# gaoxiang12/ORB-YGZ-SLAM

Hardware: AMD Instinct MI355X
Metric: frames/s ORB extract+match, 752x480 8-lvl 1000-feat; 1->8 GPU scaling (higher is better)
Workload: dtype u8

## Files before the change

### orb_ygz_slam_amd/csrc/extract_kernels.hip

```cpp
#include <cstdlib>

#include <cstring>
#include <mutex>
#include "kernels.h"
#include "wave_ops.h"
#include "describe_lds.h"
#include "fast9_quad.h"
#include "fast_lane_quads.h"
#include "orb_pattern_table.h"

namespace ygzf {

typedef short v2s __attribute__((ext_vector_type(2)));
typedef unsigned short v2u __attribute__((ext_vector_type(2)));

__device__ __forceinline__ int lane_id() { return threadIdx.x & 63; }
__device__ __forceinline__ int wave_id() { return __builtin_amdgcn_readfirstlane(threadIdx.x >> 6); }

#ifdef YGZF_PHASE_CLOCK
constexpr int kPhaseSlots = 8192;
__device__ unsigned g_phase_rec[2][kPhaseSlots][10];
struct PhaseClk {
    unsigned long long t;
    unsigned a[8], extra;
// ... 98 lines not shown
    __syncthreads();
    const unsigned long long total = tmp64[16];
    unsigned long long off = tmp64[wave_id()] + incl - s;
    for (int i = lo; i < hi; i++) {
        const unsigned long long v = (unsigned long long) (unsigned) a[i] | ((unsigned long long) (unsigned) b[i] << 21) | ((unsigned long long) (unsigned) c[i] << 42);
        a[i] = (int) (off & 0x1FFFFFu); b[i] = (int) ((off >> 21) & 0x1FFFFFu); c[i] = (int) (off >> 42);
        off += v;
    }
    __syncthreads();
    *totA = (int) (total & 0x1FFFFFu); *totB = (int) ((total >> 21) & 0x1FFFFFu); *totC = (int) (total >> 42);
}

constexpr int kRadixBits = 7;
constexpr int radix_hist_ints(int waves) { return (1 << kRadixBits) * waves; }
template <int kWaves>
__device__ void block_radix_sort(unsigned *k0, unsigned *v0, unsigned *k1, unsigned *v1, int n, int bits,
                                 volatile int *histT, int *tmp, unsigned **rk, unsigned **rv) {
    static_assert(kWaves >= 1 && kWaves <= 16, "block_excl_scan's scratch holds up to 16 waves");
    const int lane = lane_id(), wave = wave_id();
    constexpr int nw = kWaves;
    const int seg = (((n + nw - 1) / nw) + 63) & ~63;
    const int start = wave * seg;
    const int end = min(n, start + seg);
    const unsigned long long lt = (1ull << lane) - 1ull;
    constexpr int NB = 1 << kRadixBits;
    for (int shift = 0; shift < bits; shift += kRadixBits) {
        for (int t = threadIdx.x; t < NB * nw; t += blockDim.x) histT[t] = 0;
        __syncthreads();
        for (int i = start + lane; i < end; i += 64) {
            const int d = (k0[i] >> shift) & (NB - 1);
            atomicAdd((int *) &histT[d * nw + wave], 1);
        }
        __syncthreads();
        block_scan_array((int *) histT, NB * nw, tmp);
        for (int base = start; base < end; base += 64) {
            const int i = base + lane;
            const bool valid = i < end;
            const unsigned key = valid ? k0[i] : 0u;
            const unsigned val = valid ? v0[i] : 0u;
            const int d = (key >> shift) & (NB - 1);
            unsigned long long m = __ballot(valid);
// ... 945 lines not shown
    int tid, l, f, parts, part;
    LevelGeom g;
    OctShared S;
    int nCells, passEv;
    int *PS;
    unsigned *candB;
    unsigned *xTab;
    const unsigned short *cc;
    const unsigned *sl;
    unsigned *key0, *val0, *key1, *val1, *xy;
    int dm, nBins, binShift;
    int *lvlCnt, *gd, *gh;
    int *histT, *tmp, *flagA, *overflow, *cut, *head;
    unsigned long long *tmp64;
    bool hist, inLds;
    int M;
    unsigned *skeys, *svals;
    int n, cur, nE;
};

enum OctOutcome { kOctDone, kOctLeft, kOctAgainAlone, kOctAgainSorted };
__device__ __forceinline__ void oct_stamp(const OctLevel &w, long long *dbg, int k) {
    if (dbg && w.tid == 0 && w.f == 0 && w.part == 0) dbg[w.l * 8 + k] = wall_clock64();
}
__device__ __forceinline__ void oct_pass_stamp(OctLevel &w, long long *dbg, int nn) {
#ifdef YGZF_PHASE_CLOCK
    if (dbg && w.tid == 0 && w.f == 0 && w.part == 0 && w.passEv < 8) { dbg[16 * 8 + 16 + w.l * 16 + 2 * w.passEv] = nn; dbg[16 * 8 + 16 + w.l * 16 + 2 * w.passEv + 1] = wall_clock64(); w.passEv++; }
#endif
}
__device__ __forceinline__ void oct_helper_leaves(const OctLevel &w) {
// ... 23 lines not shown
    if (kGlobalNodes) S.cand = (unsigned *) dyn + Y.ints;
    else if (!kHist) S.cand = (unsigned *) dyn + oct_lds_sort_cand((int) (p - dyn), a.ldsCand);
    w.xTab = (unsigned *) (kGlobalNodes ? S.nlo[0] : dyn + Y.xTab);
}

template <int kBlock> __device__ __forceinline__ int oct_cell_prefix(const OctArgs &a, const OctLevel &w) {
    const OctShared &S = w.S;
    for (int i = w.tid; i < w.nCells; i += kBlock) S.cellPref[i] = w.cc[i];
    __syncthreads();
    const int M = block_scan_array(S.cellPref, w.nCells, w.tmp);
    if (w.tid == 0) { S.cellPref[w.nCells] = M; if (w.part == 0) a.lvlCandCnt[w.f * a.nlevels + w.l] = M; }
    __syncthreads();
    return M;
}

template <int kBlock> __device__ __forceinline__ void oct_key_tables(const OctLevel &w, int lenX, int lenY) {
    const LevelGeom &g = w.g;
    unsigned *xTab = w.xTab, *yTab = xTab + lenX, *orgTab = yTab + lenY;
    auto spread = [](unsigned v) {
        v = (v | (v << 8)) & 0x00FF00FFu;
        v = (v | (v << 4)) & 0x0F0F0F0Fu;
        v = (v | (v << 2)) & 0x33333333u;
        return (v | (v << 1)) & 0x55555555u;
    };
    auto halvings = [&](int v, int lo, int hi) {
        unsigned k = 0;
        for (int d = 0; d < g.depth; d++) {
            const int m = lo + ((hi - lo + 1) >> 1);
            const unsigned b = v >= m;
            if (b) lo = m; else hi = m;
            k = (k << 1) | b;
        }
        return k;
    };
    for (int t = w.tid; t < lenX + lenY + w.nCells; t += kBlock) {
        if (t < lenX) {
            const int root = min((int) ((float) t / g.hX), g.nIni - 1);
            xTab[t] = ((unsigned) root << (2 * g.depth)) | spread(halvings(t, (int) (g.hX * (float) root), (int) (g.hX * (float) (root + 1))));
        } else if (t < lenX + lenY) {
            yTab[t - lenX] = spread(halvings(t - lenX, 0, g.regH)) << 1;
        } else {
            const int c = t - lenX - lenY;
            const int ci = c / g.nCols, cj = c - ci * g.nCols;
            orgTab[c] = (unsigned) (cj * g.wCell) | ((unsigned) (ci * g.hCell) << 16);
        }
    }
    __syncthreads();
}

template <int kBlock> __device__ __forceinline__ void oct_path_keys(const OctLevel &w, bool useTab, int lenX, int lenY, int shares) {
    const LevelGeom &g = w.g; const OctShared &S = w.S;
    const int tid = w.tid, M = w.M, nCells = w.nCells;
    const unsigned *xTab = w.xTab, *yTab = xTab + lenX, *orgTab = yTab + lenY;
    int steps = 0;
    while ((1 << steps) < nCells) steps++;
    constexpr int kKU = 4;
    for (int i0 = tid + w.part * kKU * kBlock; i0 < M; i0 += shares * kKU * kBlock) {
        int ia[kKU], a[kKU], b[kKU];
#pragma unroll
        for (int u = 0; u < kKU; u++) { ia[u] = min(i0 + u * kBlock, M - 1); a[u] = 0; b[u] = nCells; }
        for (int st = 0; st < steps; st++) {
// ... 79 lines not shown
        int v = w.PS[b];
        for (int q = 0; q < w.parts - 1; q++) v += w.gh[(long long) q * a.histBins + b];
        w.PS[b] = v;
    }
    return kOctDone;
}

template <int kBlock> __device__ __forceinline__ void oct_order(OctLevel &w) {
    w.skeys = w.key0; w.svals = w.val0;
    if (w.hist) {
        block_scan_array(w.PS, w.nBins, w.tmp);
        if (w.tid == 0) w.PS[w.nBins] = w.M;
        __syncthreads();
    } else {
        unsigned *sk, *sv;
        block_radix_sort<kBlock / 64>(w.key0, w.val0, w.key1, w.val1, w.M, w.g.keyBits, w.histT, w.tmp, &sk, &sv);
        w.skeys = sk; w.svals = sv;
        if (w.inLds && w.candB && w.skeys == w.key1) {
            for (int i = w.tid; i < w.M; i += kBlock) { w.key0[i] = w.key1[i]; w.val0[i] = w.val1[i]; }
            __syncthreads();
            w.skeys = w.key0; w.svals = w.val0;
        }
    }
}

__device__ __forceinline__ int oct_first_bin(const int *PS, int nBins, int sh, int lo) {
    int a = 0, b = nBins >> sh;
    while (b - a > 1) {
        const int m = (a + b) >> 1;
        if (PS[m << sh] <= lo) a = m; else b = m;
    }
    return a << sh;
}
__device__ __forceinline__ void oct_bounds(const OctLevel &w, int lo, int cnt, int dep, int *a1, int *a2, int *a3) {
    if (w.hist) {
        if (dep + 1 > w.dm) {
            *w.overflow = 1;
            *a1 = *a2 = *a3 = lo + cnt;
            return;
        }
        const int sh = 2 * (w.dm - dep);
        const int f0 = oct_first_bin(w.PS, w.nBins, sh, lo), s1 = 1 << (sh - 2);
        *a1 = w.PS[f0 + s1]; *a2 = w.PS[f0 + 2 * s1]; *a3 = w.PS[f0 + 3 * s1];
    } else
        digit_bounds3(w.skeys, lo, cnt, 2 * (w.g.depth - (dep + 1)), a1, a2, a3);
}
__device__ __forceinline__ void oct_child_counts(int lo, int a1, int a2, int a3, int hi, int *k, int *e) {
    const int c0 = a1 - lo, c1 = a2 - a1, c2 = a3 - a2, c3 = hi - a3;
    *k = (c0 > 0) + (c1 > 0) + (c2 > 0) + (c3 > 0);
    *e = (c0 > 1) + (c1 > 1) + (c2 > 1) + (c3 > 1);
}
template <typename T> __device__ __forceinline__ void oct_place_children(const OctNodes &out, int lo, int cnt, int dep, int a1, int a2, int a3, int p, T *ePos, T *eCnt, int es) {
    const int bb[5] = {lo, a1, a2, a3, lo + cnt};
    int epos[4];
    for (int c = 3; c >= 0; c--) {
        const int cc2 = bb[c + 1] - bb[c];
        epos[c] = p;
        if (cc2 > 0) { out.lo[p] = bb[c]; out.cnt[p] = cc2; out.dep[p] = dep + 1; p++; }
    }
    for (int c = 0; c < 4; c++) {
        const int cc2 = bb[c + 1] - bb[c];
        if (cc2 > 1) { ePos[es] = (T) epos[c]; eCnt[es] = (T) cc2; es++; }
    }
}
__device__ __forceinline__ void oct_emit(const OctShared &S, const OctNodes &out, int lo, int cnt, int dep, int a1, int a2, int a3, int exK, int exE, int exS, int sumK) {
    if (cnt == 1) {
        const int p = sumK + exS;
        out.lo[p] = lo; out.cnt[p] = 1; out.dep[p] = dep;
    } else {
        int k, e;
        oct_child_counts(lo, a1, a2, a3, lo + cnt, &k, &e);
        oct_place_children(out, lo, cnt, dep, a1, a2, a3, sumK - (exK + k), S.Epos, S.Ecnt, exE);
    }
}
// ... 124 lines not shown
}

template <int kBlock> __device__ __forceinline__ void oct_expand_round(OctLevel &w) {
    const OctShared &S = w.S; const OctNodes in = oct_nodes(S, w.cur);
    const int tid = w.tid, n = w.n, nE = w.nE, N = w.g.nFeat;
    int seqBits = 1, cntBits = 1;
    while ((1 << seqBits) < max(nE, 2)) seqBits++;
    while ((1 << cntBits) <= w.M) cntBits++;
    for (int j = tid; j < nE; j += kBlock) { S.sk[0][j] = ((unsigned) S.Ecnt[j] << seqBits) | (unsigned) j; S.sv[0][j] = (unsigned) j; }
    for (int j = tid; j < n; j += kBlock) S.flag[j] = 0;
    if (tid == 0) *w.cut = nE - 1;
    __syncthreads();
    unsigned *ek, *ev;
    if (nE <= kBlock) { oct_rank_sort<kBlock>(w, nE); ek = S.sk[1]; ev = S.sv[1]; }
    else
        block_radix_sort<kBlock / 64>(S.sk[0], S.sv[0], S.sk[1], S.sv[1], nE, seqBits + cntBits, w.histT, w.tmp, &ek, &ev);
    for (int j = tid; j < nE; j += kBlock) {
        const int pos = S.Epos[(int) ev[nE - 1 - j]];
        const int cnt = in.cnt[pos], lo = in.lo[pos];
        int a1, a2, a3, k, e;
        oct_bounds(w, lo, cnt, in.dep[pos], &a1, &a2, &a3);
        S.b1[j] = a1; S.b2[j] = a2; S.b3[j] = a3;
        oct_child_counts(lo, a1, a2, a3, lo + cnt, &k, &e);
        S.kArr[j] = k - 1; S.eArr[j] = e;
    }
    __syncthreads();
    block_scan_array(S.kArr, nE, w.tmp);
    auto children = [&](int j) {
        const int pos = S.Epos[(int) ev[nE - 1 - j]];
        const int cnt = in.cnt[pos], lo = in.lo[pos];
        int k, e;
// ... 49 lines not shown
        const int prevSize = w.n;
        oct_full_pass<kBlock>(w);
        oct_pass_stamp(w, dbg, w.n);
        if (w.n >= N || w.n == prevSize) finish = true;
        else if (w.n + 3 * w.nE > N) toExpand = true;
    }
    while (!finish) {
        const int prevSize = w.n;
        if (w.nE == 0) break;
        oct_expand_round<kBlock>(w);
        oct_pass_stamp(w, dbg, -w.n);
        if (w.n >= N || w.n == prevSize) finish = true;
    }
}

template <bool kHist, int kBlock> __device__ __forceinline__ OctOutcome oct_attempt(const OctArgs &a, OctLevel &w, bool useHist, bool alone) {
    const LevelGeom &g = w.g; const int tid = w.tid;
    w.hist = kHist && useHist;
    if (kHist && tid == 0) *w.overflow = 0;
    w.M = oct_cell_prefix<kBlock>(a, w);
    if (w.M == 0) { oct_empty_level<kBlock>(a, w); return kOctLeft; }
    oct_stamp(w, a.dbg, 1);
    w.inLds = w.M <= a.ldsCand;
    if (w.inLds) {
        w.key0 = w.S.cand; w.val0 = w.S.cand + a.ldsCand;
        if (w.candB) { w.key1 = w.candB; w.val1 = w.candB + a.ldsCand; }
        else { w.key1 = w.S.cand + 2 * a.ldsCand; w.val1 = w.S.cand + 3 * a.ldsCand; }
    }
    const int lenX = max(g.regW, g.nCols * g.wCell) + 9, lenY = max(g.regH, g.nRows * g.hCell) + 9;
    const bool useTab = lenX + lenY + w.nCells <= oct_lds_tab_room(kHist, w.nCells, a.cap, a.regionInts) && g.depth <= 15;
    if (useTab) oct_key_tables<kBlock>(w, lenX, lenY);
    if (w.hist) {
        for (int b = tid; b <= w.nBins; b += kBlock) w.PS[b] = 0;
        __syncthreads();
    }
    const bool shared = w.hist && w.parts > 1 && !alone;
    oct_path_keys<kBlock>(w, useTab, lenX, lenY, shared ? w.parts : 1);
    if (shared) {
        const OctOutcome o = oct_hand_over<kBlock>(a, w);
        if (o != kOctDone) return o;
    }
    __syncthreads();
    oct_stamp(w, a.dbg, 2);
    oct_order<kBlock>(w);
    oct_stamp(w, a.dbg, 3);
    oct_subdivide<kBlock>(w, a.dbg);
    if (w.hist && *w.overflow) {
        __syncthreads();
        if (a.dbg && tid == 0) atomicAdd((unsigned long long *) &a.dbg[16 * 8 + w.l], 1ull);
        return kOctAgainSorted;
    }
    return kOctDone;
}

template <int kBlock> __device__ __forceinline__ void oct_best_hist(const OctLevel &w) {
    const OctShared &S = w.S; const OctNodes in = oct_nodes(S, w.cur);
    const int tid = w.tid, n = w.n, M = w.M, lane = lane_id(), wave = wave_id();
    int *PS = w.PS;
    for (int i = tid; i < n; i += kBlock) {
        const int sh = 2 * (w.dm - in.dep[i]);
        S.b1[i] = oct_first_bin(PS, w.nBins, sh, in.lo[i]);
// ... 32 lines not shown
        const bool ok = i < n;
        const int lo = ok ? in.lo[i] : 0, cnt = ok ? in.cnt[i] : 0;
        unsigned best = 0;
        for (int k = sl16; k < cnt; k += 16) best = max(best, w.svals[lo + k]);
        best = max(best, (unsigned) __builtin_amdgcn_update_dpp(0, (int) best, 0xB1, 0xF, 0xF, true));
        best = max(best, (unsigned) __builtin_amdgcn_update_dpp(0, (int) best, 0x4E, 0xF, 0xF, true));
        best = max(best, (unsigned) __builtin_amdgcn_update_dpp(0, (int) best, 0x141, 0xF, 0xF, true));
        best = max(best, (unsigned) __builtin_amdgcn_update_dpp(0, (int) best, 0x140, 0xF, 0xF, true));
        if (ok && sl16 == 0) S.kArr[i] = (int) best;
    }
}

template <int kBlock> __device__ __forceinline__ void oct_emit_keypoints(const OctArgs &a, const OctLevel &w) {
    const OctShared &S = w.S; const LevelGeom &g = w.g;
    const int tid = w.tid, n = w.n;
    unsigned *oxy = a.lvlKpXY + (long long) w.f * a.kpStride + g.kpBase;
    unsigned char *osc = a.lvlKpScore + (long long) w.f * a.kpStride + g.kpBase;
    for (int i = tid; i < n; i += kBlock) {
        const unsigned best = (unsigned) S.kArr[i];
        const unsigned idx = 0xFFFFFFu - (best & 0xFFFFFFu);
        const unsigned p = w.xy[idx];
        const unsigned kx = (p & 0xFFFFu) + kBorder, ky = (p >> 16) + kBorder;
        oxy[i] = kx | (ky << 16);
        osc[i] = (unsigned char) (best >> 24);
        S.b1[i] = (int) (kx | (ky << 16));
        S.b2[i] = (int) (best >> 24);
        S.sk[0][i] = ((ky >> 6) << 6) | (kx >> 6);
        S.sv[0][i] = (unsigned) i;
    }
    __syncthreads();
    unsigned *ok = S.sk[0], *ov = S.sv[0];
    if (gridDim.y > 4) block_radix_sort<kBlock / 64>(S.sk[0], S.sv[0], S.sk[1], S.sv[1], n, 12, w.histT, w.tmp, &ok, &ov);
    uint2 *pr = a.procRec + (long long) w.f * a.kpStride + g.kpBase;
    for (int i = tid; i < g.kpCap; i += kBlock) {
        if (i < n) {
            const unsigned li = ov[i];
            pr[i] = make_uint2((unsigned) S.b1[li], (unsigned) S.b2[li] | (li << 8) | ((unsigned) w.l << 24));
        } else pr[i] = make_uint2(0u, kNoKeypoint);
    }
    if (tid == 0) *w.lvlCnt = n;
}

template <bool kGlobalNodes, bool kHist, int kBlock>
__global__ __launch_bounds__(kBlock) __attribute__((amdgpu_waves_per_eu(kHist ? 4 : 8, 8))) void k_octree(OctArgs a) {
    static_assert(!(kGlobalNodes && kHist), "the histogram plan keeps the node arrays in LDS");
    extern __shared__ __attribute__((aligned(16))) int dyn[];
    __shared__ int histT[radix_hist_ints(kBlock / 64)];
// ... 13 lines not shown
    w.gd = kHist && w.parts > 1 ? a.gDone + (w.f * a.nlevels + w.l) : nullptr;
    w.gh = kHist && w.parts > 1 ? a.gHist + ((long long) w.f * a.nlevels + w.l) * (w.parts - 1) * a.histBins : nullptr;
    if (w.nCells <= 0 || g.nCols <= 0) { oct_empty_level<kBlock>(a, w); return; }
    oct_carve<kGlobalNodes, kHist>(a, w, dyn);
    w.cc = a.cellCnt + (long long) w.f * a.totalCells + g.cellBase;
    w.sl = a.slots + (long long) w.f * a.totalSlots + g.slotBase;
    const long long cand = (long long) w.f * a.candStride + g.candBase;
    w.key0 = a.candKey0 + cand; w.val0 = a.candVal0 + cand; w.key1 = a.candKey1 + cand; w.val1 = a.candVal1 + cand; w.xy = a.candXY + cand;
    w.dm = 0;
    if (kHist) {
        w.dm = g.depth;
        while (w.dm > 0 && ((long long) g.nIni << (2 * w.dm)) > (long long) a.histBins) w.dm--;
    }
    w.nBins = g.nIni << (2 * w.dm);
    w.binShift = 2 * (g.depth - w.dm);
    bool useHist = kHist && w.dm >= 1, alone = false;
    if (w.part != 0 && !useHist) { oct_helper_leaves(w); return; }
    for (;;) {
        const OctOutcome o = oct_attempt<kHist, kBlock>(a, w, useHist, alone);
        if (o == kOctLeft) return;
        if (o == kOctDone) break;
        if (o == kOctAgainAlone) alone = true;
        else useHist = false;
    }
    oct_stamp(w, a.dbg, 4);
    if (w.hist) oct_best_hist<kBlock>(w);
    else oct_best_sorted<kBlock>(w);
    __syncthreads();
    oct_emit_keypoints<kBlock>(a, w);
    oct_stamp(w, a.dbg, 5);
    if (a.dbg && w.tid == 0 && w.f == 0) { a.dbg[w.l * 8 + 6] = w.M; a.dbg[w.l * 8 + 7] = w.n; }
}

__device__ __forceinline__ float fast_atan2_deg(float y, float x) {
    const float k = (float) (180.0 / 3.14159265358979323846);
    const float p1 = 0.9997878412794807f * k, p3 = -0.3258083974640975f * k, p5 = 0.1555786518463281f * k,
                p7 = -0.04432655554792128f * k;
    const float ax = fabsf(x), ay = fabsf(y);
// ... 556 lines not shown
    else
        hipLaunchKernelGGL((k_fast_tab_persist<false>), grid, block, lds, st, fs, dCells, iniTh, minTh, cellCnt, slots, totalCells, totalSlots, recsPerFrame, magic,
                           totalItems, perXcd, winRows, smapRows, quadCap, stats, counters);
}

hipError_t octree_prepare(size_t ldsBytes, bool globalNodes, bool hist) {
    constexpr int kOctMaxDyn = 160 * 1024 - 10 * 1024;
    if (hist) return hipFuncSetAttribute((const void *) k_octree<false, true, kOctBlock>, hipFuncAttributeMaxDynamicSharedMemorySize, kOctMaxDyn);
    if (globalNodes) return hipFuncSetAttribute((const void *) k_octree<true, false, kOctBlock>, hipFuncAttributeMaxDynamicSharedMemorySize, kOctMaxDyn);
    hipError_t e = hipFuncSetAttribute((const void *) k_octree<false, false, 1024>, hipFuncAttributeMaxDynamicSharedMemorySize, kOctMaxDyn);
    if (e == hipSuccess) e = hipFuncSetAttribute((const void *) k_octree<false, false, 512>, hipFuncAttributeMaxDynamicSharedMemorySize, kOctMaxDyn);
    if (e == hipSuccess) e = hipFuncSetAttribute((const void *) k_octree<false, false, 256>, hipFuncAttributeMaxDynamicSharedMemorySize, kOctMaxDyn);
    return e;
}

void launch_octree(hipStream_t st, const OctArgs &a, int nLaunchLevels, int nFrames, size_t ldsBytes, int block, int helpers) {
    const dim3 grid(nLaunchLevels, nFrames, helpers);
    switch (a.histBins > 0 ? 1 : a.nodeArena ? 2 : block) {
        case 1: hipLaunchKernelGGL((k_octree<false, true, kOctBlock>), grid, dim3(kOctBlock), ldsBytes, st, a); break;
        case 2: hipLaunchKernelGGL((k_octree<true, false, kOctBlock>), grid, dim3(kOctBlock), ldsBytes, st, a); break;
        case 256: hipLaunchKernelGGL((k_octree<false, false, 256>), grid, dim3(256), ldsBytes, st, a); break;
        case 512: hipLaunchKernelGGL((k_octree<false, false, 512>), grid, dim3(512), ldsBytes, st, a); break;
        default: hipLaunchKernelGGL((k_octree<false, false, 1024>), grid, dim3(1024), ldsBytes, st, a); break;
    }
}

void launch_describe(hipStream_t st, const FrameSet &fs, const LevelGeom *dGeom, int nlevels, const int *lvlKpCnt, int *lvlBase,
                     const uint2 *procRec, int kpStride, ygzf_kp *outKp, uint8_t *outDesc, int *outCnt, int outStride, int nFrames, int cvMode) {
    const bool own = nFrames <= 4;
    if (!own) hipLaunchKernelGGL(k_level_bases, dim3((nFrames + 255) / 256), dim3(256), 0, st, lvlKpCnt, nlevels, nFrames, lvlBase, outCnt);
// ... 80 lines not shown
```

### orb_ygz_slam_amd/csrc/kernels.h

```cpp
#ifndef YGZF_KERNELS_H
#define YGZF_KERNELS_H
#include "ygzf_internal.h"
#include "ygzf_remap_plan.h"
#include "lds_layout.h"

namespace ygzf {

hipError_t upload_constants(const int *umax16);

struct PyrTabs {
    const int *xofs;
    const short *xalpha;
    const int *yofs;
    const short *ybeta;
    const PyrColRec *cols;
    const PyrRowRec *rows;
    const PyrTileRec *tiles;
};
void launch_pyr_resize(hipStream_t st, const FrameSet &fs, const LevelGeom *dGeom, const LevelGeom &g, int level, int nFrames, const PyrTabs &T);
constexpr int kPyrFolds = 4;
__host__ __device__ constexpr int pyr_fold_chunks(int foldLog2) { return foldLog2 == 0 ? 21 : foldLog2 == 1 ? 11 : foldLog2 == 2 ? 6 : 3; }
__host__ __device__ constexpr int pyr_fold_pitch(int foldLog2) { return 16 * pyr_fold_chunks(foldLog2); }
__host__ __device__ constexpr int pyr_fold_rows(int foldLog2) { return foldLog2 == 0 ? 44 : foldLog2 == 1 ? 84 : foldLog2 == 2 ? 166 : 330; }
constexpr int kPyrTileRows = 32;
// ... 32 lines not shown
void launch_pack_results(hipStream_t st, const int *cnt, const ygzf_kp *kp, const uint8_t *desc, int nFrames, int kpStride, void *dst, size_t offKp, size_t offDesc);
void launch_pack_levels(hipStream_t st, const FrameSet &fs, const LevelGeom *dGeom, int firstLevel, int nlevels, const unsigned *offsets, uint8_t *dst);
void launch_fast_cells(hipStream_t st, const FrameSet &fs, const LevelGeom *dGeom, int nlevels, int iniTh, int minTh,
                       unsigned short *cellCnt, unsigned *slots, int totalCells, long long totalSlots, int totalGroups, int smapRows,
                       int nFrames, int winPitch, int winRows, int quadCap, const int *groupBaseHost, bool iniFirst, unsigned *stats);
constexpr int kFastTabMaxCell = 41;
void launch_fast_tab(hipStream_t st, const FrameSet &fs, const FastCellRec *dCells, int iniTh, int minTh, unsigned short *cellCnt, unsigned *slots,
                     int totalCells, long long totalSlots, int totalGroups, int smapRows, int nFrames, int winRows, int quadCap, bool iniFirst,
                     unsigned *stats);
hipError_t phase_clocks_read(int kernel, unsigned long long *out16, bool reset);
constexpr size_t kFastPersistCounterBytes = 64 * 256;
void launch_fast_tab_persist(hipStream_t st, const FrameSet &fs, const FastCellRec *dCells, int iniTh, int minTh, unsigned short *cellCnt, unsigned *slots,
                             int totalCells, long long totalSlots, int totalGroups, int smapRows, int nFrames, int winRows, int quadCap, bool iniFirst,
                             unsigned *stats, unsigned *counters, int nWorkgroups);
constexpr int kFastStatWords = 8 * 64;
int octree_lds_cand(int maxCellsPerLevel, int cap, size_t budget);
hipError_t octree_prepare(size_t ldsBytes, bool globalNodes, bool hist);
struct OctArgs {
    const LevelGeom *geom;
    int nlevels, levelBase;
    const unsigned short *cellCnt;
    const unsigned *slots;
    int totalCells;
    long long totalSlots;
    unsigned *candKey0, *candVal0, *candKey1, *candVal1, *candXY;
    long long candStride;
    unsigned *lvlKpXY;
    unsigned char *lvlKpScore;
    int *lvlKpCnt, *lvlCandCnt;
    uint2 *procRec;
    int kpStride;
    int cap, ldsCand;
    int *nodeArena;
    int regionInts, histBins;
    int *gHist, *gDone;
    int doneTarget, spinBudget;
    long long *dbg;
};
void launch_octree(hipStream_t st, const OctArgs &a, int nLaunchLevels, int nFrames, size_t ldsBytes, int block, int helpers);
constexpr int kOctDbgAlone = 16 * 8 + 16 + 16 * 16;
constexpr int kOctDbgAloneFrames = kOctDbgAlone + 16;
constexpr int kOctDbgWords = kOctDbgAloneFrames + 1;
void launch_describe(hipStream_t st, const FrameSet &fs, const LevelGeom *dGeom, int nlevels, const int *lvlKpCnt, int *lvlBase,
                     const uint2 *procRec, int kpStride, ygzf_kp *outKp, uint8_t *outDesc, int *outCnt, int outStride, int nFrames, int cvMode);
void launch_hamming_pairs(hipStream_t st, const void *a, const void *b, int n, int *out);

struct MatchQueryScratch;
struct MatchArgs {
// ... 374 lines not shown
```

### orb_ygz_slam_amd/csrc/ygzf_api.hip

```cpp
#include <cmath>
#include <cstdarg>
#include <cstdio>
#include <cstdlib>
#include <cstring>
#include <limits>
#include <mutex>

#include "ygzf_ctx.h"

using namespace ygzf;

thread_local std::string g_create_err;

int apply_geometry(ygzf_ctx *c, int w, int h, int nFrames) {
    if (w < 1 || h < 1) return fail(c, YGZF_ERR_INVALID, "image size %dx%d", w, h);
    if (w > c->maxW || h > c->maxH) return fail(c, YGZF_ERR_INVALID, "image %dx%d exceeds the context maximum %dx%d", w, h, c->maxW, c->maxH);
    if (nFrames < 1 || nFrames > c->maxBatch) return fail(c, YGZF_ERR_INVALID, "batch of %d frames (context maximum %d)", nFrames, c->maxBatch);
    const int L = c->tab.cfg.nlevels;
    if (c->geo.w != w || c->geo.h != h) {
        Geometry G;
        OctPlan oct;
        std::string msg;
        int rc = build_geometry(c->tab, c->pins, w, h, G, &msg);
        if (!rc) rc = plan_octree(G, L, c->pins, oct, &msg);
// ... 37 lines not shown
                for (size_t q = 0; q < rel.size(); q++) {
                    std::memset(&rel[q], 0, sizeof rel[q]);
                    for (int l = G.pyrBase; l < L; l++) rel[q].lv[l - G.pyrBase] = G.pyrPlan[q].lv[l];
                }
                HIPCHECK(c, hipMemcpy(c->dPyrPlan.p, lv, sizeof lv, hipMemcpyHostToDevice));
                HIPCHECK(c, hipMemcpy((char *) c->dPyrPlan.p + sizeof G.pyrLevels, rel.data(), rel.size() * sizeof(PyrStripPlan), hipMemcpyHostToDevice));
            }
            if (pyr_strips_prepare(G.pyrStripLds) != hipSuccess) {
                (void) hipGetLastError();
                G.pyrPlan.clear();
            }
        }
        rc = ensure(c, c->dFastCells, std::max<size_t>(G.fastCells.size() * sizeof(FastCellRec), 32));
        if (rc) return rc;
        if (!G.fastCells.empty()) HIPCHECK(c, hipMemcpy(c->dFastCells.p, G.fastCells.data(), G.fastCells.size() * sizeof(FastCellRec), hipMemcpyHostToDevice));
        if (oct.haveSmall || oct.kind == OctPlan::Hist) HIPCHECK(c, octree_prepare(0, false, true));
        if (oct.kind != OctPlan::Hist) HIPCHECK(c, octree_prepare(oct.launches[0].lds, oct.launches[0].arena, false));
        c->oct = oct;
        c->geo = G;
    }
    const Geometry &G = c->geo;
    const size_t B = (size_t) nFrames;
    int rc = 0;
    const size_t oldPyr = c->dPyr.bytes;
    rc = ensure(c, c->dPyr, std::max<size_t>(B * G.pyrBytes, 16) + 256);
    if (oldPyr != c->dPyr.bytes) forget_image(c);
    if (rc) return rc;
    if ((rc = ensure(c, c->dCellCnt, std::max<size_t>(B * G.totalCells * sizeof(unsigned short), 16)))) return rc;
    if ((rc = ensure(c, c->dSlots, std::max<size_t>(B * G.totalSlots * sizeof(unsigned), 16)))) return rc;
    const size_t cb = std::max<size_t>(B * G.candStride * sizeof(unsigned), 16);
// ... 127 lines not shown
    }
    if (collect) HIPCHECK(c, hipMemcpyAsync(c->hFastStats, c->dFastStats.p, kFastStatWords * sizeof(unsigned), hipMemcpyDeviceToHost, c->stream));
    return YGZF_OK;
}

static OctArgs oct_args(const ygzf_ctx *c, const OctLaunch &grp, long long *odbg) {
    const Geometry &G = c->geo;
    OctArgs a{};
    a.geom = (const LevelGeom *) c->dGeom.p; a.nlevels = c->tab.cfg.nlevels; a.levelBase = grp.l0; a.cap = grp.cap; a.dbg = odbg;
    a.cellCnt = (const unsigned short *) c->dCellCnt.p; a.slots = (const unsigned *) c->dSlots.p; a.totalCells = G.totalCells; a.totalSlots = G.totalSlots;
    a.candKey0 = (unsigned *) c->dK0.p; a.candVal0 = (unsigned *) c->dV0.p; a.candKey1 = (unsigned *) c->dK1.p; a.candVal1 = (unsigned *) c->dV1.p;
    a.candXY = (unsigned *) c->dXY.p; a.candStride = G.candStride; a.procRec = (uint2 *) c->dProcOrder.p; a.kpStride = G.kpStride;
    a.lvlKpXY = (unsigned *) c->dLvlXY.p; a.lvlKpScore = (unsigned char *) c->dLvlScore.p; a.lvlKpCnt = (int *) c->dLvlCnt.p; a.lvlCandCnt = (int *) c->dLvlCand.p;
    a.ldsCand = grp.ldsCand; a.regionInts = grp.regionInts; a.histBins = grp.histBins;
    a.nodeArena = grp.arena ? (int *) c->dOctNodes.p : nullptr;
    return a;
}

static int arm_oct_helpers(ygzf_ctx *c, int nFrames, int L, const OctLaunch &small, OctArgs *a, int *helpersOut) {
    const Geometry &G = c->geo;
    int helpers = c->pins.octHelpers;
    if (helpers < 0) helpers = G.totalCells >= 2000 ? std::min(8, std::max(1, c->cuCount) / std::max(1, nFrames * L)) : 1;
    helpers = std::max(1, std::min(helpers, std::min(8, std::max(1, c->cuCount / std::max(1, nFrames * L)))));
    if (helpers > 1) {
        const size_t words = (size_t) nFrames * L * (helpers - 1) * small.histBins, bytes = (words + 64) * sizeof(int) + (size_t) nFrames * L * sizeof(int);
        int rcH = ensure(c, c->dOctHist, bytes);
        if (rcH) return rcH;
        const ygzf_ctx::OctHistLayout lay{nFrames, helpers, small.histBins, c->dOctHist.bytes};
        if (!(lay == c->octHistLayout) || c->octDoneTarget > (1 << 30)) {
            HIPCHECK(c, hipMemsetAsync((int *) c->dOctHist.p + words, 0, c->dOctHist.bytes - words * sizeof(int), c->stream));
// ... 29 lines not shown
        for (const auto &grp : plan.launches) fprintf(stderr, " levels %d-%d cap %d bins %d lds %zu;", grp.l0, grp.l0 + grp.n - 1, grp.cap, grp.histBins, grp.lds);
        fprintf(stderr, " workgroups of %d frames that fell back to the sort, per level:", nFrames);
        for (int l = 0; l < L; l++) fprintf(stderr, " %lld", st[16 * 8 + l]);
        fprintf(stderr, "]\n");
    }
    if (!smallHelpers && plan.kind == OctPlan::SortGroups) {
        fprintf(stderr, "[ygzf octree sort plan: %zu launches;", plan.launches.size());
        for (const auto &grp : plan.launches)
            fprintf(stderr, " levels %d-%d threads %d cap %d candidates %d lds %zu;", grp.l0, grp.l0 + grp.n - 1, grp.block, grp.cap, grp.ldsCand, grp.lds);
        fprintf(stderr, "]\n");
    }
    if (!smallHelpers && plan.kind == OctPlan::SortOne) {
        const OctLaunch &one = plan.launches[0];
        fprintf(stderr, "[ygzf octree single launch: levels 0-%d cap %d candidates %d lds %zu node arrays in %s]\n", L - 1, one.cap, one.ldsCand, one.lds,
                one.arena ? "the arena" : "lds");
    }
    if (smallHelpers) {
        fprintf(stderr, "[ygzf octree small plan: %d frames, %d workgroups per level; workgroups 0 that gave up waiting for their helpers, per level:", nFrames, smallHelpers);
        for (int l = 0; l < L; l++) fprintf(stderr, " %lld", st[kOctDbgAlone + l]);
        fprintf(stderr, "; frames mask 0x%llx]\n", (unsigned long long) st[kOctDbgAloneFrames]);
    }
    return YGZF_OK;
}

int run_extract(ygzf_ctx *c, const FrameSet &fs, int nFrames, bool pyramidReady) {
    const Geometry &G = c->geo;
    pyramid_taken(c);
    const int L = c->tab.cfg.nlevels;
    int rc;
    queue_carry(c, false);
// ... 760 lines not shown
```

### orb_ygz_slam_amd/csrc/ygzf_ctx.h

```cpp
#ifndef YGZF_CTX_H
#define YGZF_CTX_H
#include <cmath>
#include <cstdarg>
#include <cstdio>
#include <cstdlib>
#include <cstring>
#include <limits>
#include <mutex>
#include <set>
#include <type_traits>
#include <unordered_map>

#include "ygzf_plan.h"

namespace ygzf {
enum KernelKind { KK_PYR = 0, KK_FAST, KK_OCTREE, KK_DESCRIBE, KK_HAMMING, KK_BACKPROJ, KK_MATCH, KK_SIA, KK_FAST10, KK_DSO, KK_STEREO, KK_DIRECT, KK_BOW, KK_FRUSTUM, KK_DISTINCTIVE, KK_BOWNODES, KK_GRID, KK_FASTQ, KK_TRI, KK_FASTP, KK_FUSE, KK_PROJ, KK_BOWKF, KK_KFDB, KK_KFGRID, KK_COUNT };
static const char *kKernelNames[KK_COUNT] = {"k_pyr_resize", "k_fast_tab", "k_octree", "k_describe", "k_hamming_pairs",
                                             "k_backproject_unit", "k_match_last", "k_sia_run", "k_f10_*", "k_dso_cells", "k_stereo_*", "k_direct_projection", "k_bow_descend", "k_frustum", "k_distinctive", "k_bow_nodes", "k_features_in_area", "k_fast_quads", "k_tri_nodes", "k_fast_tab_persist", "k_fuse", "k_proj_search", "k_bow_kf_nodes", "k_kfdb_query", "k_kf_grid_build"};

}

using namespace ygzf;

struct Held {
// ... 62 lines not shown
    bool alignCarry = false;
    std::vector<unsigned char> alKey;
    int identityPoses = 0;
    void *identityPosesPtr = nullptr;
    PlanPins pins = PlanPins::from_env();
    OctPlan oct;
    bool carryOff = false;
    struct OctHistLayout {
        int frames = 0, helpers = 0, histBins = 0;
        size_t bytes = 0;
        bool operator==(const OctHistLayout &o) const { return frames == o.frames && helpers == o.helpers && histBins == o.histBins && bytes == o.bytes; }
    } octHistLayout;
    int octDoneTarget = 0;
    static constexpr int octSmallWgs = 128;
    Buf dOctNodes;
    int fastPlan = 0;
    bool fastIniFirst = false;
    unsigned fastLaunches = 0;
    double fastExtraRounds = 0.0;
    double fastCornerQuadsPerRun = 0.0, fastRunsPerCell = 0.0;
    Buf dFastStats;
    Buf dFastCells;
    Buf dMatchStat;
    Buf dPack;
    int fastKernel = 0;
    unsigned *hFastStats = nullptr;
    Buf dFastCtr;
    int cuCount = 256;
    Buf dResPack;
    Buf dUpStage;
// ... 303 lines not shown
```

### orb_ygz_slam_amd/csrc/ygzf_plan.h

```cpp
#ifndef YGZF_PLAN_H
#define YGZF_PLAN_H
#include "kernels.h"

#define YGZF_HIDDEN __attribute__((visibility("hidden")))

namespace ygzf {
YGZF_HIDDEN int cv_round_host(double v);
static inline int align_up(int v, int a) { return (v + a - 1) / a * a; }

struct Geometry {
    int w = 0, h = 0;
    std::vector<LevelGeom> lv;
    std::vector<int> xofs, yofs;
    std::vector<short> xalpha, ybeta;
    std::vector<PyrColRec> pyrCols;
    std::vector<PyrRowRec> pyrRows;
    std::vector<PyrTileRec> pyrTiles;
    long long pyrBytes = 0;
    std::vector<PyrStripPlan> pyrPlan;
    int pyrStripOffA = 0, pyrStripOffB = 0;
    int pyrBase = 0;
    PyrStripLevel pyrLevels[kMaxLevels];
    size_t pyrStripLds = 0;
    int totalCells = 0, maxCellsPerLevel = 0;
// ... 1 lines not shown
    int fastWCellMax = 1;
    std::vector<FastCellRec> fastCells;
    long long totalSlots = 0;
    long long candStride = 0;
    int kpStride = 0, kpCapMax = 0;
};

struct PlanPins {
    int pyrStrips = 0;
    int pyrStripBase = 0;
    int pyrStripFrames = 16;
    bool octOneGroup = false;
    int octBlock = 0;
    size_t octLdsBytes = 0;
    enum OctPlanPin { Auto, Hist, Sort } octPlan = Auto;
    int octHistBins = 0;
    int octHelpers = -1, octHelperSpin = 1 << 16;
    int fastPersist = -1, fastPersistWgs = 8;
    static PlanPins from_env() {
        PlanPins p;
        p.pyrStrips = (int) forced("pyr_strips", p.pyrStrips);
        p.pyrStripBase = (int) forced("pyr_strip_base", p.pyrStripBase);
        p.pyrStripFrames = (int) forced("pyr_strip_frames", p.pyrStripFrames);
        p.octOneGroup = forced("oct_groups", 0) == 1;
        p.octBlock = (int) forced("oct_block", p.octBlock);
        p.octLdsBytes = (size_t) forced("oct_lds_kb", 0) * 1024;
        p.octPlan = forced_is("oct_plan", "hist") ? Hist : forced_is("oct_plan", "sort") ? Sort : Auto;
        p.octHistBins = (int) forced("oct_hist_bins", p.octHistBins);
        p.octHelpers = (int) forced("oct_helpers", p.octHelpers);
        p.octHelperSpin = (int) forced("oct_helper_spin", p.octHelperSpin);
        p.fastPersist = (int) forced("fast_persist", p.fastPersist);
        p.fastPersistWgs = (int) forced("fast_persist_wgs", p.fastPersistWgs);
        return p;
    }
};

YGZF_HIDDEN int build_geometry(const Tables &T, const PlanPins &pins, int w, int h, Geometry &G, std::string *err);

struct OctLaunch {
    int l0 = 0, n = 0, block = kOctBlock, cap = 0, ldsCand = 0, regionInts = 0, histBins = 0;
    size_t lds = 0;
    bool arena = false;
};
struct OctPlan {
    enum Kind { SortGroups, SortOne, Hist } kind = SortOne;
    std::vector<OctLaunch> launches;
    bool haveSmall = false;
    OctLaunch small;
};
YGZF_HIDDEN std::vector<OctLaunch> plan_oct_sort(const Geometry &G, int L, bool oneGroup, int block, size_t ldsBytes);
YGZF_HIDDEN int plan_octree(const Geometry &G, int L, const PlanPins &pins, OctPlan &plan, std::string *err);

struct FastChoice {
    enum Kind { Quads, Tab, Persist } kind;
    int resident;
};
YGZF_HIDDEN FastChoice choose_fast(const Geometry &G, int fastKernelSetting, const PlanPins &pins, int cuCount, int nFrames, size_t tabLds);

}
#endif
```

### orb_ygz_slam_amd/csrc/ygzf_plan.hip

```cpp
#include "ygzf_plan.h"

#include <algorithm>
#include <cmath>
#include <cstdarg>
#include <cstdio>
#include <cstring>

namespace ygzf {

int cv_round_host(double v) { return (int) std::nearbyint(v); }

void Tables::init(const ygzf_extractor_cfg &c) {
    cfg = c;
    const int L = c.nlevels;
    scale.assign(L, 1.f);
    sigma2.assign(L, 1.f);
    invScale.assign(L, 1.f);
    invSigma2.assign(L, 1.f);
    for (int i = 1; i < L; i++) {
        scale[i] = scale[i - 1] * c.scale_factor;
        sigma2[i] = scale[i] * scale[i];
    }
    for (int i = 0; i < L; i++) {
        invScale[i] = 1.0f / scale[i];
// ... 381 lines not shown
    if (plan.kind != OctPlan::Hist) {
        const size_t lds = oct_lds_bytes(arena ? kOctLdsArena : kOctLdsSort, G.maxCellsPerLevel, G.kpCapMax, ldsCand, 0, 0);
        if (lds > 150 * 1024)
            return plan_fail(err, YGZF_ERR_UNSUPPORTED, "octree kernel needs %zu bytes of LDS (cells/level %d, list cap %d)", lds, G.maxCellsPerLevel, G.kpCapMax);
        if (!arena && ldsCand > 0) {
            plan.kind = OctPlan::SortGroups;
            plan.launches = plan_oct_sort(G, L, pins.octOneGroup, pins.octBlock, pins.octLdsBytes);
        } else {
            OctLaunch one;
            one.n = L; one.cap = G.kpCapMax; one.ldsCand = ldsCand; one.lds = lds; one.arena = arena;
            plan.kind = OctPlan::SortOne;
            plan.launches.push_back(one);
        }
    }
    if (pins.octPlan != PlanPins::Sort) plan.haveSmall = size_oct_hist_group(G, 0, L, pins.octHistBins, true, &plan.small);
    return YGZF_OK;
}

FastChoice choose_fast(const Geometry &G, int fastKernelSetting, const PlanPins &pins, int cuCount, int nFrames, size_t tabLds) {
    const bool tab = fastKernelSetting != YGZF_FAST_KERNEL_REGISTER_STAGING && G.fastWCellMax <= kFastTabMaxCell && G.pyrBytes < (1ll << 32) &&
                     G.w < 65536 && G.h < 65536 && G.totalSlots < (1ll << 32);
    const size_t fastLds = tab ? tabLds : 0;
    const int perCu = tab ? (int) std::min<size_t>((size_t) pins.fastPersistWgs, (size_t) (160 * 1024) / std::max<size_t>(fastLds, 1)) : 0;
    const int resident = perCu * cuCount;
    const int persistMode = pins.fastPersist;
    const bool persist = tab && resident > 0 && (long long) nFrames * G.totalGroups >= 64 &&
                         (persistMode == 1 || (persistMode != 0 && G.totalGroups >= 1000 && (long long) nFrames * G.totalGroups >= 4LL * resident));
    return FastChoice{persist ? FastChoice::Persist : tab ? FastChoice::Tab : FastChoice::Quads, resident};
}

// ... 75 lines not shown
```

Baseline: 285,700.

## Sort octree keys by top radix digits only and precompute key tables once

The octree sort now radix-sorts only the top two 7-bit digits of the Morton keys. It falls back to a full sort when subdivision needs finer bits than were sorted. The per-level key lookup tables are built once by a setup kernel and copied into LDS instead of being recomputed in every workgroup, and the keypoint tile sort uses only as many bits as there are tiles. The aim is fewer radix passes and less redundant table arithmetic per frame, at the risk of extra restart passes when clusters require deeper subdivision.

New measurement: 292,500 (median of 6 runs). +2.4%, better.

```diff
diff --git a/orb_ygz_slam_amd/csrc/extract_kernels.hip b/orb_ygz_slam_amd/csrc/extract_kernels.hip
--- a/orb_ygz_slam_amd/csrc/extract_kernels.hip
+++ b/orb_ygz_slam_amd/csrc/extract_kernels.hip
@@ -136,7 +136,7 @@
 constexpr int kRadixBits = 7;
 constexpr int radix_hist_ints(int waves) { return (1 << kRadixBits) * waves; }
 template <int kWaves>
-__device__ void block_radix_sort(unsigned *k0, unsigned *v0, unsigned *k1, unsigned *v1, int n, int bits,
+__device__ void block_radix_sort(unsigned *k0, unsigned *v0, unsigned *k1, unsigned *v1, int n, int shift0, int bits,
                                  volatile int *histT, int *tmp, unsigned **rk, unsigned **rv) {
     static_assert(kWaves >= 1 && kWaves <= 16, "block_excl_scan's scratch holds up to 16 waves");
     const int lane = lane_id(), wave = wave_id();
@@ -146,7 +146,7 @@
     const int end = min(n, start + seg);
     const unsigned long long lt = (1ull << lane) - 1ull;
     constexpr int NB = 1 << kRadixBits;
-    for (int shift = 0; shift < bits; shift += kRadixBits) {
+    for (int shift = shift0; shift < bits; shift += kRadixBits) {
         for (int t = threadIdx.x; t < NB * nw; t += blockDim.x) histT[t] = 0;
         __syncthreads();
         for (int i = start + lane; i < end; i += 64) {
@@ -1122,6 +1122,7 @@
     int *histT, *tmp, *flagA, *overflow, *cut, *head;
     unsigned long long *tmp64;
     bool hist, inLds;
+    int lowBit;
     int M;
     unsigned *skeys, *svals;
     int n, cur, nE;
@@ -1175,9 +1176,8 @@
     return M;
 }
 
-template <int kBlock> __device__ __forceinline__ void oct_key_tables(const OctLevel &w, int lenX, int lenY) {
-    const LevelGeom &g = w.g;
-    unsigned *xTab = w.xTab, *yTab = xTab + lenX, *orgTab = yTab + lenY;
+__device__ __forceinline__ void oct_key_tables_write(const LevelGeom &g, int lenX, int lenY, int nCells, unsigned *xTab, int tid, int stride) {
+    unsigned *yTab = xTab + lenX, *orgTab = yTab + lenY;
     auto spread = [](unsigned v) {
         v = (v | (v << 8)) & 0x00FF00FFu;
         v = (v | (v << 4)) & 0x0F0F0F0Fu;
@@ -1194,7 +1194,7 @@
         }
         return k;
     };
-    for (int t = w.tid; t < lenX + lenY + w.nCells; t += kBlock) {
+    for (int t = tid; t < lenX + lenY + nCells; t += stride) {
         if (t < lenX) {
             const int root = min((int) ((float) t / g.hX), g.nIni - 1);
             xTab[t] = ((unsigned) root << (2 * g.depth)) | spread(halvings(t, (int) (g.hX * (float) root), (int) (g.hX * (float) (root + 1))));
@@ -1206,6 +1206,17 @@
             orgTab[c] = (unsigned) (cj * g.wCell) | ((unsigned) (ci * g.hCell) << 16);
         }
     }
+}
+struct OctTabOffsets { int off[kMaxLevels]; };
+__global__ __launch_bounds__(256) void k_oct_key_tables(const LevelGeom *__restrict__ geom, OctTabOffsets offs, unsigned *__restrict__ tabs) {
+    const LevelGeom g = geom[blockIdx.x];
+    if (threadIdx.x == 0) tabs[blockIdx.x] = (unsigned) offs.off[blockIdx.x];
+    if (g.nCols <= 0 || g.nRows <= 0) return;
+    oct_key_tables_write(g, oct_tab_len_x(g), oct_tab_len_y(g), g.nCols * g.nRows, tabs + offs.off[blockIdx.x], (int) threadIdx.x, (int) blockDim.x);
+}
+template <int kBlock> __device__ __forceinline__ void oct_key_tables(const OctArgs &a, const OctLevel &w, int lenX, int lenY) {
+    const unsigned *src = a.keyTabs + a.keyTabs[w.l];
+    for (int t = w.tid; t < lenX + lenY + w.nCells; t += kBlock) w.xTab[t] = src[t];
     __syncthreads();
 }
 
@@ -1315,7 +1326,7 @@
         __syncthreads();
     } else {
         unsigned *sk, *sv;
-        block_radix_sort<kBlock / 64>(w.key0, w.val0, w.key1, w.val1, w.M, w.g.keyBits, w.histT, w.tmp, &sk, &sv);
+        block_radix_sort<kBlock / 64>(w.key0, w.val0, w.key1, w.val1, w.M, w.lowBit, w.g.keyBits, w.histT, w.tmp, &sk, &sv);
         w.skeys = sk; w.svals = sv;
         if (w.inLds && w.candB && w.skeys == w.key1) {
             for (int i = w.tid; i < w.M; i += kBlock) { w.key0[i] = w.key1[i]; w.val0[i] = w.val1[i]; }
@@ -1343,8 +1354,15 @@
         const int sh = 2 * (w.dm - dep);
         const int f0 = oct_first_bin(w.PS, w.nBins, sh, lo), s1 = 1 << (sh - 2);
         *a1 = w.PS[f0 + s1]; *a2 = w.PS[f0 + 2 * s1]; *a3 = w.PS[f0 + 3 * s1];
-    } else
-        digit_bounds3(w.skeys, lo, cnt, 2 * (w.g.depth - (dep + 1)), a1, a2, a3);
+    } else {
+        const int shift = 2 * (w.g.depth - (dep + 1));
+        if (shift < w.lowBit) {
+            *w.overflow = 1;
+            *a1 = *a2 = *a3 = lo + cnt;
+            return;
+        }
+        digit_bounds3(w.skeys, lo, cnt, shift, a1, a2, a3);
+    }
 }
 __device__ __forceinline__ void oct_child_counts(int lo, int a1, int a2, int a3, int hi, int *k, int *e) {
     const int c0 = a1 - lo, c1 = a2 - a1, c2 = a3 - a2, c3 = hi - a3;
@@ -1354,11 +1372,13 @@
 template <typename T> __device__ __forceinline__ void oct_place_children(const OctNodes &out, int lo, int cnt, int dep, int a1, int a2, int a3, int p, T *ePos, T *eCnt, int es) {
     const int bb[5] = {lo, a1, a2, a3, lo + cnt};
     int epos[4];
+#pragma unroll
     for (int c = 3; c >= 0; c--) {
         const int cc2 = bb[c + 1] - bb[c];
         epos[c] = p;
         if (cc2 > 0) { out.lo[p] = bb[c]; out.cnt[p] = cc2; out.dep[p] = dep + 1; p++; }
     }
+#pragma unroll
     for (int c = 0; c < 4; c++) {
         const int cc2 = bb[c + 1] - bb[c];
         if (cc2 > 1) { ePos[es] = (T) epos[c]; eCnt[es] = (T) cc2; es++; }
@@ -1513,7 +1533,7 @@
     unsigned *ek, *ev;
     if (nE <= kBlock) { oct_rank_sort<kBlock>(w, nE); ek = S.sk[1]; ev = S.sv[1]; }
     else
-        block_radix_sort<kBlock / 64>(S.sk[0], S.sv[0], S.sk[1], S.sv[1], nE, seqBits + cntBits, w.histT, w.tmp, &ek, &ev);
+        block_radix_sort<kBlock / 64>(S.sk[0], S.sv[0], S.sk[1], S.sv[1], nE, 0, seqBits + cntBits, w.histT, w.tmp, &ek, &ev);
     for (int j = tid; j < nE; j += kBlock) {
         const int pos = S.Epos[(int) ev[nE - 1 - j]];
         const int cnt = in.cnt[pos], lo = in.lo[pos];
@@ -1593,10 +1613,11 @@
     }
 }
 
-template <bool kHist, int kBlock> __device__ __forceinline__ OctOutcome oct_attempt(const OctArgs &a, OctLevel &w, bool useHist, bool alone) {
+template <bool kHist, int kBlock> __device__ __forceinline__ OctOutcome oct_attempt(const OctArgs &a, OctLevel &w, bool useHist, bool alone, bool fullSort) {
     const LevelGeom &g = w.g; const int tid = w.tid;
     w.hist = kHist && useHist;
-    if (kHist && tid == 0) *w.overflow = 0;
+    w.lowBit = !kHist && a.sortPrefix && !fullSort && g.keyBits > 2 * kRadixBits ? g.keyBits - 2 * kRadixBits : 0;
+    if (tid == 0) *w.overflow = 0;
     w.M = oct_cell_prefix<kBlock>(a, w);
     if (w.M == 0) { oct_empty_level<kBlock>(a, w); return kOctLeft; }
     oct_stamp(w, a.dbg, 1);
@@ -1606,9 +1627,9 @@
         if (w.candB) { w.key1 = w.candB; w.val1 = w.candB + a.ldsCand; }
         else { w.key1 = w.S.cand + 2 * a.ldsCand; w.val1 = w.S.cand + 3 * a.ldsCand; }
     }
-    const int lenX = max(g.regW, g.nCols * g.wCell) + 9, lenY = max(g.regH, g.nRows * g.hCell) + 9;
+    const int lenX = oct_tab_len_x(g), lenY = oct_tab_len_y(g);
     const bool useTab = lenX + lenY + w.nCells <= oct_lds_tab_room(kHist, w.nCells, a.cap, a.regionInts) && g.depth <= 15;
-    if (useTab) oct_key_tables<kBlock>(w, lenX, lenY);
+    if (useTab) oct_key_tables<kBlock>(a, w, lenX, lenY);
     if (w.hist) {
         for (int b = tid; b <= w.nBins; b += kBlock) w.PS[b] = 0;
         __syncthreads();
@@ -1621,9 +1642,20 @@
     }
     __syncthreads();
     oct_stamp(w, a.dbg, 2);
-    oct_order<kBlock>(w);
-    oct_stamp(w, a.dbg, 3);
-    oct_subdivide<kBlock>(w, a.dbg);
+    for (;;) {
+        oct_order<kBlock>(w);
+        oct_stamp(w, a.dbg, 3);
+        oct_subdivide<kBlock>(w, a.dbg);
+        if (w.lowBit == 0 || !*w.overflow) break;
+        __syncthreads();
+        if (tid == 0) {
+            *w.overflow = 0;
+            if (a.dbg) atomicAdd((unsigned long long *) &a.dbg[16 * 8 + w.l], 1ull);
+        }
+        w.lowBit = 0;
+        w.key0 = w.skeys; w.val0 = w.svals;
+        __syncthreads();
+    }
     if (w.hist && *w.overflow) {
         __syncthreads();
         if (a.dbg && tid == 0) atomicAdd((unsigned long long *) &a.dbg[16 * 8 + w.l], 1ull);
@@ -1686,6 +1718,9 @@
 template <int kBlock> __device__ __forceinline__ void oct_emit_keypoints(const OctArgs &a, const OctLevel &w) {
     const OctShared &S = w.S; const LevelGeom &g = w.g;
     const int tid = w.tid, n = w.n;
+    const int tilesX = (g.w + 63) >> 6, tilesY = (g.h + 63) >> 6;
+    int tileBits = 0;
+    while ((1 << tileBits) < tilesX * tilesY) tileBits++;
     unsigned *oxy = a.lvlKpXY + (long long) w.f * a.kpStride + g.kpBase;
     unsigned char *osc = a.lvlKpScore + (long long) w.f * a.kpStride + g.kpBase;
     for (int i = tid; i < n; i += kBlock) {
@@ -1697,12 +1732,12 @@
         osc[i] = (unsigned char) (best >> 24);
         S.b1[i] = (int) (kx | (ky << 16));
         S.b2[i] = (int) (best >> 24);
-        S.sk[0][i] = ((ky >> 6) << 6) | (kx >> 6);
+        S.sk[0][i] = (ky >> 6) * (unsigned) tilesX + (kx >> 6);
         S.sv[0][i] = (unsigned) i;
     }
     __syncthreads();
     unsigned *ok = S.sk[0], *ov = S.sv[0];
-    if (gridDim.y > 4) block_radix_sort<kBlock / 64>(S.sk[0], S.sv[0], S.sk[1], S.sv[1], n, 12, w.histT, w.tmp, &ok, &ov);
+    if (gridDim.y > 4) block_radix_sort<kBlock / 64>(S.sk[0], S.sv[0], S.sk[1], S.sv[1], n, 0, tileBits, w.histT, w.tmp, &ok, &ov);
     uint2 *pr = a.procRec + (long long) w.f * a.kpStride + g.kpBase;
     for (int i = tid; i < g.kpCap; i += kBlock) {
         if (i < n) {
@@ -1746,14 +1781,14 @@
     }
     w.nBins = g.nIni << (2 * w.dm);
     w.binShift = 2 * (g.depth - w.dm);
-    bool useHist = kHist && w.dm >= 1, alone = false;
+    bool useHist = kHist && w.dm >= 1, alone = false, fullSort = false;
     if (w.part != 0 && !useHist) { oct_helper_leaves(w); return; }
     for (;;) {
-        const OctOutcome o = oct_attempt<kHist, kBlock>(a, w, useHist, alone);
+        const OctOutcome o = oct_attempt<kHist, kBlock>(a, w, useHist, alone, fullSort);
         if (o == kOctLeft) return;
         if (o == kOctDone) break;
         if (o == kOctAgainAlone) alone = true;
-        else useHist = false;
+        else { useHist = false; fullSort = true; }
     }
     oct_stamp(w, a.dbg, 4);
     if (w.hist) oct_best_hist<kBlock>(w);
@@ -2340,6 +2375,12 @@
     return e;
 }
 
+void launch_oct_key_tables(hipStream_t st, const LevelGeom *dGeom, int nlevels, const int *offHost, unsigned *tabs) {
+    OctTabOffsets offs{};
+    for (int l = 0; l < nlevels && l < kMaxLevels; l++) offs.off[l] = offHost[l];
+    hipLaunchKernelGGL(k_oct_key_tables, dim3(nlevels), dim3(256), 0, st, dGeom, offs, tabs);
+}
+
 void launch_octree(hipStream_t st, const OctArgs &a, int nLaunchLevels, int nFrames, size_t ldsBytes, int block, int helpers) {
     const dim3 grid(nLaunchLevels, nFrames, helpers);
     switch (a.histBins > 0 ? 1 : a.nodeArena ? 2 : block) {
diff --git a/orb_ygz_slam_amd/csrc/kernels.h b/orb_ygz_slam_amd/csrc/kernels.h
--- a/orb_ygz_slam_amd/csrc/kernels.h
+++ b/orb_ygz_slam_amd/csrc/kernels.h
@@ -70,6 +70,10 @@
                              int totalCells, long long totalSlots, int totalGroups, int smapRows, int nFrames, int winRows, int quadCap, bool iniFirst,
                              unsigned *stats, unsigned *counters, int nWorkgroups);
 constexpr int kFastStatWords = 8 * 64;
+__host__ __device__ inline int oct_tab_len_x(const LevelGeom &g) { return (g.regW > g.nCols * g.wCell ? g.regW : g.nCols * g.wCell) + 9; }
+__host__ __device__ inline int oct_tab_len_y(const LevelGeom &g) { return (g.regH > g.nRows * g.hCell ? g.regH : g.nRows * g.hCell) + 9; }
+__host__ __device__ inline int oct_tab_words(const LevelGeom &g) { return g.nCols <= 0 || g.nRows <= 0 ? 0 : oct_tab_len_x(g) + oct_tab_len_y(g) + g.nCols * g.nRows; }
+void launch_oct_key_tables(hipStream_t st, const LevelGeom *dGeom, int nlevels, const int *offHost, unsigned *tabs);
 int octree_lds_cand(int maxCellsPerLevel, int cap, size_t budget);
 hipError_t octree_prepare(size_t ldsBytes, bool globalNodes, bool hist);
 struct OctArgs {
@@ -88,6 +92,8 @@
     int kpStride;
     int cap, ldsCand;
     int *nodeArena;
+    int sortPrefix;
+    const unsigned *keyTabs;
     int regionInts, histBins;
     int *gHist, *gDone;
     int doneTarget, spinBudget;
diff --git a/orb_ygz_slam_amd/csrc/ygzf_api.hip b/orb_ygz_slam_amd/csrc/ygzf_api.hip
--- a/orb_ygz_slam_amd/csrc/ygzf_api.hip
+++ b/orb_ygz_slam_amd/csrc/ygzf_api.hip
@@ -75,6 +75,10 @@
         rc = ensure(c, c->dFastCells, std::max<size_t>(G.fastCells.size() * sizeof(FastCellRec), 32));
         if (rc) return rc;
         if (!G.fastCells.empty()) HIPCHECK(c, hipMemcpy(c->dFastCells.p, G.fastCells.data(), G.fastCells.size() * sizeof(FastCellRec), hipMemcpyHostToDevice));
+        rc = ensure(c, c->dOctKeyTabs, std::max<size_t>((size_t) oct.keyTabWords * sizeof(unsigned), 16));
+        if (rc) return rc;
+        launch_oct_key_tables(c->stream, (const LevelGeom *) c->dGeom.p, L, oct.keyTabOff, (unsigned *) c->dOctKeyTabs.p);
+        HIPCHECK(c, hipGetLastError());
         if (oct.haveSmall || oct.kind == OctPlan::Hist) HIPCHECK(c, octree_prepare(0, false, true));
         if (oct.kind != OctPlan::Hist) HIPCHECK(c, octree_prepare(oct.launches[0].lds, oct.launches[0].arena, false));
         c->oct = oct;
@@ -232,6 +236,8 @@
     a.lvlKpXY = (unsigned *) c->dLvlXY.p; a.lvlKpScore = (unsigned char *) c->dLvlScore.p; a.lvlKpCnt = (int *) c->dLvlCnt.p; a.lvlCandCnt = (int *) c->dLvlCand.p;
     a.ldsCand = grp.ldsCand; a.regionInts = grp.regionInts; a.histBins = grp.histBins;
     a.nodeArena = grp.arena ? (int *) c->dOctNodes.p : nullptr;
+    a.sortPrefix = c->pins.octSortPrefix && !grp.arena && grp.histBins == 0;
+    a.keyTabs = (const unsigned *) c->dOctKeyTabs.p;
     return a;
 }
 
@@ -291,6 +297,12 @@
         const OctLaunch &one = plan.launches[0];
         fprintf(stderr, "[ygzf octree single launch: levels 0-%d cap %d candidates %d lds %zu node arrays in %s]\n", L - 1, one.cap, one.ldsCand, one.lds,
                 one.arena ? "the arena" : "lds");
+    }
+    if (!smallHelpers && plan.kind != OctPlan::Hist) {
+        const bool prefix = c->pins.octSortPrefix && !plan.launches[0].arena;
+        fprintf(stderr, "[ygzf octree key order: %s; workgroups of %d frames that started over with the full sort, per level:", prefix ? "prefix" : "full", nFrames);
+        for (int l = 0; l < L; l++) fprintf(stderr, " %lld", st[16 * 8 + l]);
+        fprintf(stderr, "]\n");
     }
     if (smallHelpers) {
         fprintf(stderr, "[ygzf octree small plan: %d frames, %d workgroups per level; workgroups 0 that gave up waiting for their helpers, per level:", nFrames, smallHelpers);
diff --git a/orb_ygz_slam_amd/csrc/ygzf_ctx.h b/orb_ygz_slam_amd/csrc/ygzf_ctx.h
--- a/orb_ygz_slam_amd/csrc/ygzf_ctx.h
+++ b/orb_ygz_slam_amd/csrc/ygzf_ctx.h
@@ -100,6 +100,7 @@
     int octDoneTarget = 0;
     static constexpr int octSmallWgs = 128;
     Buf dOctNodes;
+    Buf dOctKeyTabs;
     int fastPlan = 0;
     bool fastIniFirst = false;
     unsigned fastLaunches = 0;
diff --git a/orb_ygz_slam_amd/csrc/ygzf_plan.h b/orb_ygz_slam_amd/csrc/ygzf_plan.h
--- a/orb_ygz_slam_amd/csrc/ygzf_plan.h
+++ b/orb_ygz_slam_amd/csrc/ygzf_plan.h
@@ -39,6 +39,7 @@
     int octBlock = 0;
     size_t octLdsBytes = 0;
     enum OctPlanPin { Auto, Hist, Sort } octPlan = Auto;
+    bool octSortPrefix = true;
     int octHistBins = 0;
     int octHelpers = -1, octHelperSpin = 1 << 16;
     int fastPersist = -1, fastPersistWgs = 8;
@@ -51,6 +52,7 @@
         p.octBlock = (int) forced("oct_block", p.octBlock);
         p.octLdsBytes = (size_t) forced("oct_lds_kb", 0) * 1024;
         p.octPlan = forced_is("oct_plan", "hist") ? Hist : forced_is("oct_plan", "sort") ? Sort : Auto;
+        p.octSortPrefix = forced_is("oct_sort", "full") ? false : forced_is("oct_sort", "prefix") ? true : p.octSortPrefix;
         p.octHistBins = (int) forced("oct_hist_bins", p.octHistBins);
         p.octHelpers = (int) forced("oct_helpers", p.octHelpers);
         p.octHelperSpin = (int) forced("oct_helper_spin", p.octHelperSpin);
@@ -72,6 +74,8 @@
     std::vector<OctLaunch> launches;
     bool haveSmall = false;
     OctLaunch small;
+    int keyTabOff[kMaxLevels] = {0};
+    int keyTabWords = 0;
 };
 YGZF_HIDDEN std::vector<OctLaunch> plan_oct_sort(const Geometry &G, int L, bool oneGroup, int block, size_t ldsBytes);
 YGZF_HIDDEN int plan_octree(const Geometry &G, int L, const PlanPins &pins, OctPlan &plan, std::string *err);
diff --git a/orb_ygz_slam_amd/csrc/ygzf_plan.hip b/orb_ygz_slam_amd/csrc/ygzf_plan.hip
--- a/orb_ygz_slam_amd/csrc/ygzf_plan.hip
+++ b/orb_ygz_slam_amd/csrc/ygzf_plan.hip
@@ -419,6 +419,11 @@
         }
     }
     if (pins.octPlan != PlanPins::Sort) plan.haveSmall = size_oct_hist_group(G, 0, L, pins.octHistBins, true, &plan.small);
+    plan.keyTabWords = kMaxLevels;
+    for (int l = 0; l < L; l++) {
+        plan.keyTabOff[l] = plan.keyTabWords;
+        plan.keyTabWords += (oct_tab_words(G.lv[l]) + 3) & ~3;
+    }
     return YGZF_OK;
 }
 
```
